# Streampunk/phaneron

Hardware: AMD Instinct MI355X
Metric: frames/sec, 4-layer 2160p50 composite pipeline (v210 unpack->CSC->combine->CSC->v210 pack) (higher is better)
Workload: dtype f32

## Files before the change

include/phaneron_hip.h:

```cpp
#ifndef PHANERON_HIP_H
#define PHANERON_HIP_H

#include <stddef.h>
#include <stdint.h>

#ifdef __cplusplus
extern "C" {
#endif

#define PH_ABI_VERSION 8

enum {
  PH_OK = 0,
  PH_E_INVALID = -1,
  PH_E_NO_DEVICE = -2,
  PH_E_HIP = -3,
  PH_E_UNKNOWN_KERNEL = -4,
  PH_E_RANGE = -5
};

typedef struct ph_ctx ph_ctx;
typedef struct ph_buf ph_buf;
typedef struct ph_program ph_program;

// ... 248 lines not shown
int ph_chan_compose_multi(ph_ctx *ctx, int queue, int n, const ph_chan_layer *layers, int n_out, const ph_chan_output *outs,
                          uint32_t out_width, uint32_t out_height, const void *rd_col_matrix12, const void *rd_gamma_lut,
                          const void *rd_gamut9);
int ph_compose_up_write_multi(ph_ctx *ctx, int queue, int jobs, int n, const ph_image_layer *const *layer_sets, int n_out,
                              const ph_chan_output *outs, uint32_t out_width, uint32_t out_height);

int ph_lut_register(ph_ctx *ctx, const void *device_lut_f32, const float *host_lut65536);
int ph_lut_unregister(ph_ctx *ctx, const void *device_lut_f32);
int ph_lut_query(ph_ctx *ctx, const void *device_lut_f32, uint32_t *lds_bytes, uint32_t *index_bias,
                 uint32_t *blocks_per_octave_log2);
typedef struct ph_lut_layout {
  uint32_t lds_bytes, hole, delta_off, shift, index_bias;
  float a_scale;
} ph_lut_layout;
int ph_lut_layout_of(const float *host_lut65536, ph_lut_layout *layout, void *lds_image, size_t capacity);
int ph_ctx_set_option(ph_ctx *ctx, const char *name, int value);

int ph_colour_gamma2linear_lut(const char *colspec, float *lut65536);
int ph_colour_linear2gamma_lut(const char *colspec, float *lut65536);
int ph_colour_ycbcr2rgb_matrix(const char *colspec, int num_bits, int luma_black, int luma_white,
                               int chroma_range, float *m12);
int ph_colour_rgb2ycbcr_matrix(const char *colspec, int num_bits, int luma_black, int luma_white,
                               int chroma_range, float *m12);
int ph_colour_rgb2rgb_matrix(const char *src_colspec, const char *dst_colspec, float *m9);
int ph_transform_matrix(int width, int height, int flip_h, int flip_v, double anchor_x,
                        double anchor_y, double scale_x, double scale_y, double offset_x,
                        double offset_y, double rotate, float *m9);

int ph_abi_version(void);

// ... 5 lines not shown
```

phaneron_amd/capi.py:

```python
import ctypes as C
import os
import sys

import numpy as np

_HERE = os.path.dirname(os.path.abspath(__file__))
LIB_PATH = os.environ.get("PHANERON_HIP_LIB") or os.path.join(_HERE, "lib", "libphaneron_hip.so")

QUEUE_LOAD, QUEUE_PROCESS, QUEUE_UNLOAD = 0, 1, 2
HOST_READONLY, HOST_WRITEONLY, HOST_NONE = 0, 1, 2
ARG_BUF, ARG_U32, ARG_I32, ARG_F32 = 0, 1, 2, 3

EXPORTS = [
    "ph_abi_version", "ph_last_error", "ph_ctx_create", "ph_ctx_destroy", "ph_ctx_info", "ph_ctx_stream",
    "ph_wait_finish", "ph_buf_create", "ph_buf_wrap", "ph_buf_addref", "ph_buf_release", "ph_buf_refcount",
    "ph_buf_bytes", "ph_buf_device_ptr", "ph_buf_dims", "ph_buf_host_access", "ph_buf_host_ptr",
    "ph_ctx_buffer_stats", "ph_program_create", "ph_program_destroy", "ph_program_kernel", "ph_run_program", "ph_check_program", "ph_chan_compose", "ph_yadif_pair_packed",
    "ph_v210_pitch_bytes", "ph_v210_read", "ph_v210_read_batch", "ph_v210_write", "ph_yadif", "ph_yadif_pair", "ph_v210_yadif_pair", "ph_transform", "ph_resize", "ph_combine",
    "ph_transition_dissolve", "ph_transition_wipe", "ph_mixer", "ph_wipe", "ph_fused_v210_combine",
    "ph_colour_gamma2linear_lut", "ph_colour_linear2gamma_lut", "ph_colour_ycbcr2rgb_matrix",
    "ph_colour_rgb2ycbcr_matrix", "ph_colour_rgb2rgb_matrix", "ph_transform_matrix",
    "ph_lut_register", "ph_lut_unregister", "ph_lut_query", "ph_lut_layout_of", "ph_compose_up_write_v210_pair", "ph_compose_up_write_v210_batch", "ph_pack_read_batch", "ph_ctx_set_option", "ph_compose_write_v210", "ph_compose_wipe_write_v210",
    "ph_pack_plane_bytes", "ph_pack_read", "ph_pack_write", "ph_queue_wait_queue", "ph_buf_download_async",
    "ph_event_record", "ph_event_wait", "ph_event_query", "ph_event_destroy", "ph_queue_query",
    "ph_graph_begin", "ph_graph_end", "ph_graph_launch", "ph_graph_destroy", "ph_fused_v210_combine_batch",
    "ph_program_resolve", "ph_route_unique_id", "ph_route_init", "ph_route_destroy", "ph_route_group_begin",
    "ph_route_group_end", "ph_route_send", "ph_route_recv", "ph_route_after_queue", "ph_queue_after_route",
    "ph_route_wait", "ph_route_stream", "ph_route_comm_count", "ph_chan_compose_v210", "ph_chan_compose_batch", "ph_run_programs", "ph_event_record_timed", "ph_event_elapsed_us", "ph_ctx_host_pool_stats",
    "ph_v210_yadif_pair_fmt", "ph_compose_up_write_v210", "ph_trace_begin", "ph_trace_end", "ph_run_programs_progress", "ph_buf_reuse", "ph_image_unpack_rgb",
    "ph_chan_compose_multi", "ph_compose_up_write_multi",
]


class PhaneronError(RuntimeError):
    pass


class _ArgVal(C.Union):
    _fields_ = [("buf", C.c_void_p), ("u32", C.c_uint32), ("i32", C.c_int32), ("f32", C.c_float)]


class PhArg(C.Structure):
    _fields_ = [("name", C.c_char_p), ("kind", C.c_int), ("v", _ArgVal)]


# ... 117 lines not shown
        "ph_transition_wipe": (ci, [vp, ci, vp, vp, vp, ci, ci, vp]),
        "ph_mixer": (ci, [vp, ci, vp, vp, cf, ci, ci, vp]),
        "ph_wipe": (ci, [vp, ci, vp, vp, cf, ci, ci, vp]),
        "ph_fused_v210_combine": (ci, [vp, ci, ci, C.POINTER(vp), vp, cu, cu, vp, vp, vp, vp, vp]),
        "ph_fused_v210_combine_batch": (ci, [vp, ci, ci, ci, C.POINTER(vp), C.POINTER(vp), cu, cu, vp, vp, vp, vp, vp]),
        "ph_colour_gamma2linear_lut": (ci, [C.c_char_p, f32p]),
        "ph_colour_linear2gamma_lut": (ci, [C.c_char_p, f32p]),
        "ph_colour_ycbcr2rgb_matrix": (ci, [C.c_char_p, ci, ci, ci, ci, f32p]),
        "ph_colour_rgb2ycbcr_matrix": (ci, [C.c_char_p, ci, ci, ci, ci, f32p]),
        "ph_colour_rgb2rgb_matrix": (ci, [C.c_char_p, C.c_char_p, f32p]),
        "ph_transform_matrix": (ci, [ci, ci, ci, ci, cd, cd, cd, cd, cd, cd, cd, f32p]),
        "ph_lut_register": (ci, [vp, vp, f32p]),
        "ph_lut_unregister": (ci, [vp, vp]),
        "ph_lut_query": (ci, [vp, vp, C.POINTER(cu), C.POINTER(cu), C.POINTER(cu)]),
        "ph_lut_layout_of": (ci, [f32p, C.POINTER(LutLayout), vp, C.c_size_t]),
        "ph_compose_up_write_v210_pair": (ci, [vp, ci, ci, C.POINTER(PhImageLayer), C.POINTER(PhImageLayer), vp, vp, cu, cu, cu, vp, vp]),
        "ph_compose_up_write_v210_batch": (ci, [vp, ci, ci, ci, C.POINTER(C.POINTER(PhImageLayer)), C.POINTER(vp), cu, cu, cu, vp, vp]),
        "ph_pack_read_batch": (ci, [vp, ci, ci, ci, C.POINTER(vp * 3), C.POINTER(vp), cu, cu, vp, vp, vp]),
        "ph_ctx_set_option": (ci, [vp, C.c_char_p, ci]),
        "ph_pack_plane_bytes": (ci, [ci, cu, cu, C.POINTER(cs)]),
        "ph_pack_read": (ci, [vp, ci, ci, C.POINTER(vp), vp, cu, cu, vp, vp, vp]),
        "ph_pack_write": (ci, [vp, ci, ci, vp, C.POINTER(vp), cu, cu, cu, vp, vp]),
        "ph_compose_write_v210": (ci, [vp, ci, ci, C.POINTER(PhLayer), vp, cu, cu, cu, vp, vp]),
        "ph_compose_wipe_write_v210": (ci, [vp, ci, ci, C.POINTER(PhLayer), C.POINTER(PhLayerWipe), vp, cu, cu, cu, vp, vp]),
        "ph_compose_up_write_v210": (ci, [vp, ci, ci, C.POINTER(PhImageLayer), vp, cu, cu, cu, vp, vp]),
        "ph_chan_compose_v210": (ci, [vp, ci, ci, C.POINTER(PhChanLayer), vp, cu, cu, cu, vp, vp, vp, vp, vp]),
        "ph_chan_compose": (ci, [vp, ci, ci, C.POINTER(PhChanLayer), ci, C.POINTER(C.c_void_p), cu, cu, cu, vp, vp, vp, vp, vp]),
        "ph_chan_compose_batch": (ci, [vp, ci, ci, C.POINTER(PhChanJob), cu, cu, vp, vp, vp, vp, vp]),
        "ph_chan_compose_multi": (ci, [vp, ci, ci, C.POINTER(PhChanLayer), ci, C.POINTER(PhChanOutput), cu, cu, vp, vp, vp]),
        "ph_compose_up_write_multi": (ci, [vp, ci, ci, ci, C.POINTER(C.POINTER(PhImageLayer)), ci, C.POINTER(PhChanOutput), cu, cu]),
# ... 57 lines not shown
def lut_layout(lut):
    lut = np.ascontiguousarray(lut, np.float32)
    assert lut.shape == (65536,)
    lay = LutLayout()
    n = lib().ph_lut_layout_of(lut, C.byref(lay), None, 0)
    if n < 0:
        check(n)
    if n == 0:
        return None, None
    image = np.zeros(n, np.uint8)
    if lib().ph_lut_layout_of(lut, C.byref(lay), image.ctypes.data_as(C.c_void_p), n) != n:
        check(-1)
    return {k: getattr(lay, k) for k, _ in LutLayout._fields_}, image


def gamma2linear_lut(colspec):
    out = np.empty(65536, np.float32)
    check(lib().ph_colour_gamma2linear_lut(colspec.encode(), out))
    return out


def linear2gamma_lut(colspec):
    out = np.empty(65536, np.float32)
    check(lib().ph_colour_linear2gamma_lut(colspec.encode(), out))
    return out


def ycbcr2rgb_matrix(colspec, num_bits=10, luma_black=64, luma_white=940, chroma_range=896):
    out = np.empty(12, np.float32)
    check(lib().ph_colour_ycbcr2rgb_matrix(colspec.encode(), num_bits, luma_black, luma_white, chroma_range, out))
# ... 659 lines not shown
```

phaneron_amd/csrc/ph_api.cpp:

```cpp
#include <atomic>
#include <chrono>
#include <cstdarg>
#include <cstdio>
#include <cstring>
#include <dlfcn.h>
#include <map>
#include <mutex>
#include <string>
#include <vector>

#include "../../include/phaneron_hip.h"
#include "ph_internal.h"
#include "ph_kernels.h"
#include "ph_lut_host.h"

using ph::KernelId;
using namespace ph;

namespace {
thread_local std::string g_err;
}

int fail(int code, const char *fmt, ...) {
  char buf[512];
// ... 831 lines not shown
int ph_lut_layout_of(const float *host, ph_lut_layout *layout, void *lds_image, size_t capacity) {
  if (!host || !layout) return fail(PH_E_INVALID, "ph_lut_layout_of: NULL argument");
  std::vector<uint32_t> blob;
  ph::LutHostInfo info;
  memset(layout, 0, sizeof(*layout));
  if (!ph::lut_compress(host, ph::kLutMaxLdsBytes, blob, info)) return 0;
  const ph::LutView v = ph::lut_view(info, nullptr);
  layout->lds_bytes = info.bytes, layout->hole = info.hole, layout->delta_off = info.delta_off, layout->shift = info.shift;
  layout->index_bias = (uint32_t)info.bias, layout->a_scale = v.a_scale;
  if (lds_image) {
    if (capacity < info.bytes) return fail(PH_E_INVALID, "ph_lut_layout_of: the image needs %u bytes, %zu given", info.bytes, capacity);
    memset(lds_image, 0, info.hole);
    memcpy(static_cast<char *>(lds_image) + info.hole, blob.data(), info.bytes - info.hole);
  }
  return (int)info.bytes;
}

int ph_lut_query(ph_ctx *ctx, const void *dev, uint32_t *lds_bytes, uint32_t *toe, uint32_t *shift) {
  if (!ctx) return fail(PH_E_INVALID, "ph_lut_query: ctx is NULL");
  std::lock_guard<std::mutex> lock(ctx->mu);
  auto it = ctx->luts.find(dev);
  const bool have = it != ctx->luts.end();
  if (lds_bytes) *lds_bytes = have ? it->second.view.bytes : 0;
  if (toe) *toe = have ? (uint32_t)it->second.view.bias : 0;
  if (shift) *shift = have ? 23 - it->second.view.shift : 0;
  return PH_OK;
}

int ph_ctx_set_option(ph_ctx *ctx, const char *name, int value) {
  if (!ctx || !name) return fail(PH_E_INVALID, "ph_ctx_set_option: NULL argument");
// ... 1205 lines not shown
```

phaneron_amd/csrc/ph_kernels.h:

```cpp
#pragma once
#include <hip/hip_runtime.h>
#include <stddef.h>
#include <stdint.h>

#include "ph_formats.h"
#include "ph_lut.h"

namespace ph {

constexpr int kMaxLayers = 8;
constexpr int kMaxDynamicLds = 160 * 1024;

extern thread_local uint32_t t_stream_images;
extern thread_local uint32_t t_stream_threshold_mb;
static inline uint32_t image_nt(size_t bytes) {
  return t_stream_images == 2 ? (bytes > ((size_t)t_stream_threshold_mb << 20) ? 1u : 0u) : t_stream_images;
}

struct FusedArgs {
  const void *layers[kMaxLayers];
  void *out;
  uint32_t quads_per_line_used;
  uint32_t quads_per_line_pitch;
  uint32_t total_quads;
  const float *rd_cm, *rd_lut, *rd_gm, *wr_cm, *wr_lut;
  uint32_t tail_px, magic_qpp;
};

constexpr int kMaxBatch = 8;
struct FusedLdsArgs {
  FusedArgs f;
  LutView rd, wr;
  uint32_t jobs, wg_per_job;
  const void *more_layers[kMaxBatch - 1][kMaxLayers];
  void *more_out[kMaxBatch - 1];
};

struct ComposeArgs {
  const void *layers[kMaxLayers];
  const float *matrix[kMaxLayers];
  const void *wipe_with[kMaxLayers], *wipe_mask[kMaxLayers];
  int lw[kMaxLayers], lh[kMaxLayers];
  int n;
  void *out;
  uint32_t out_w, out_h, lines, first_line, line_step;
  const float *wr_cm;
  LutView wr;
};

enum : uint32_t { kChanNone = 0, kChanV210 = 1, kChanRgba = 2, kChanP10 = 3, kChanP8x422 = 4, kChanP8x420 = 5, kChanNv12 = 6, kChanP10x420 = 7,
                  kChanP010 = 8, kChanRgba8 = 9, kChanBgra8 = 10, kChanPlanarLast = kChanP010 };
// ... 215 lines not shown
```

phaneron_amd/csrc/ph_kernels_deint.hip:

```cpp
#include "ph_device.h"
#include "ph_kernels.h"
#include "ph_ldslut.h"
#include "ph_yadif.h"

#include <type_traits>

#pragma clang fp contract(off)

namespace ph {

constexpr int kDeintCols = 64 - 6;
#ifndef PH_DEINT_BLOCK
#define PH_DEINT_BLOCK 1024
#endif
constexpr int kDeintBlock = PH_DEINT_BLOCK;

struct Rgb {
  float r, g, b;
};

struct LanePick {
  uint32_t off_y, off_cb, off_cr;
  uint32_t sy, scb, scr;
};
// ... 51 lines not shown

__device__ __forceinline__ float lane_tap(float v, uint32_t lane, int d) {
  return __int_as_float(__builtin_amdgcn_ds_bpermute((int)((lane + (uint32_t)d) << 2), __float_as_int(v)));
}

#define PH_RGB(v, c) ((c) == 0 ? (v).r : (c) == 1 ? (v).g : (v).b)
#ifndef PH_DEINT_PRICE_INDEX
#define PH_DEINT_PRICE_INDEX 0
#endif

template <int TFF, bool STD, int PACK = PH_FMT_V210>
__device__ __forceinline__ void v210_yadif_pair_body(const DeintArgs &a, const ReadK &k, const LutK &lk) {
  const uint32_t wave = __builtin_amdgcn_readfirstlane(threadIdx.x >> 6), lane = threadIdx.x & 63;
  const int w = (int)a.width, h = (int)a.height;
  const uint32_t tasks = (uint32_t)a.n * a.strips * a.col_blocks;
  for (uint32_t t = blockIdx.x * (kDeintBlock / 64) + wave; t < tasks; t += gridDim.x * (kDeintBlock / 64)) {
    const uint32_t cb = t % a.col_blocks, rest = t / a.col_blocks, strip = rest % a.strips, l = rest / a.strips;
    constexpr bool V210 = PACK == PH_FMT_V210;
    const uint32_t line_bytes = V210 ? a.quads_pitch * 16u : a.quads_pitch * (fmt_wide(PACK) ? 2u : 1u);
    const int frame_bytes = (int)(line_bytes * a.height);
    auto planes = [&](const uint4 *y, const void *u, const void *v) __attribute__((always_inline)) {
      FramePlanes f;
      f.y = __builtin_amdgcn_make_buffer_rsrc(const_cast<uint4 *>(y), 0, frame_bytes, 0x00020000);
      if (fmt_cbcr(PACK)) {
        f.u = f.v = __builtin_amdgcn_make_buffer_rsrc(const_cast<void *>(u), 0, (int)(line_bytes * ((a.height + 1u) >> 1)), 0x00020000);
      } else if (!V210) {
        const int chroma_bytes = fmt_v420(PACK) ? (int)((line_bytes >> 1) * ((a.height + 1u) >> 1)) : frame_bytes / 2;
        f.u = __builtin_amdgcn_make_buffer_rsrc(const_cast<void *>(u), 0, chroma_bytes, 0x00020000);
        f.v = __builtin_amdgcn_make_buffer_rsrc(const_cast<void *>(v), 0, chroma_bytes, 0x00020000);
      } else {
        f.u = f.v = f.y;
// ... 92 lines not shown
hipError_t launch_v210_yadif_pair(hipStream_t s, DeintArgs a, int tff, uint32_t num_cus) {
  const uint32_t slots = num_cus * (kDeintBlock / 64);
  a.col_blocks = (a.width + kDeintCols - 1) / kDeintCols;
  uint32_t best_r = 16;
  uint64_t best_cost = ~0ull;
  for (uint32_t r = 8; r <= 64; r += 2) {
    const uint32_t strips = (a.height + r - 1) / r;
    const uint64_t tasks = (uint64_t)a.n * strips * a.col_blocks, rounds = (tasks + slots - 1) / slots;
    const uint64_t cost = rounds * (r + 4);
    if (cost < best_cost) best_cost = cost, best_r = r;
  }
  a.nt = image_nt((size_t)a.width * a.height * (a.rgb12 ? 12 : 16));
  a.rows_per_strip = best_r;
  a.strips = (a.height + best_r - 1) / best_r;
  const uint32_t tasks = (uint32_t)a.n * a.strips * a.col_blocks;
  const uint32_t want = (tasks + kDeintBlock / 64 - 1) / (kDeintBlock / 64);
  const uint32_t grid = want < num_cus ? want : num_cus;
  auto go = [&](auto kernel) -> hipError_t {
    hipError_t e = hipFuncSetAttribute(reinterpret_cast<const void *>(kernel), hipFuncAttributeMaxDynamicSharedMemorySize, kMaxDynamicLds);
    if (e != hipSuccess) return e;
    kernel<<<grid, kDeintBlock, a.lut.bytes, s>>>(a);
    return hipGetLastError();
  };
  switch (a.pack) {
    case PH_FMT_V210: return tff ? go(v210_yadif_pair_kernel<1, PH_FMT_V210>) : go(v210_yadif_pair_kernel<0, PH_FMT_V210>);
    case PH_FMT_YUV422P10: return tff ? go(v210_yadif_pair_kernel<1, PH_FMT_YUV422P10>) : go(v210_yadif_pair_kernel<0, PH_FMT_YUV422P10>);
    case PH_FMT_YUV422P8: return tff ? go(v210_yadif_pair_kernel<1, PH_FMT_YUV422P8>) : go(v210_yadif_pair_kernel<0, PH_FMT_YUV422P8>);
    case PH_FMT_YUV420P: return tff ? go(v210_yadif_pair_kernel<1, PH_FMT_YUV420P>) : go(v210_yadif_pair_kernel<0, PH_FMT_YUV420P>);
    case PH_FMT_NV12: return tff ? go(v210_yadif_pair_kernel<1, PH_FMT_NV12>) : go(v210_yadif_pair_kernel<0, PH_FMT_NV12>);
  }
  return hipErrorInvalidValue;
}
// ... 3 lines not shown
```

phaneron_amd/csrc/ph_kernels_fmt.hip:

```cpp
#include <cstdlib>
#include <type_traits>

#include "ph_kernels.h"
#include "ph_ldslut.h"

#pragma clang fp contract(off)

namespace ph {

constexpr int kFmtBlock = 256;

template <typename LUT>
__device__ __forceinline__ float4 yuv_to_rgba(float y, float u, float v, const ReadK &k, const LUT &lut) {
  const float r = lut.at_unit(dot4(y, u, v, 1.0f, k.r));
  const float g = lut.at_unit(dot4(y, u, v, 1.0f, k.g));
  const float b = lut.at_unit(dot4(y, u, v, 1.0f, k.b));
  return make_float4(dot3(r, g, b, k.gm[0], k.gm[1], k.gm[2]), dot3(r, g, b, k.gm[3], k.gm[4], k.gm[5]),
                     dot3(r, g, b, k.gm[6], k.gm[7], k.gm[8]), 1.0f);
}

struct FmtReadArgs {
  const void *p0, *p1, *p2;
  float4 *out;
  uint32_t width, lines, pitch;
// ... 86 lines not shown
      const float4 px = a.in[(size_t)line * a.width + x];
      const float r = lut.at_unit(px.x), gg = lut.at_unit(px.y), b = lut.at_unit(px.z);
      const uint32_t r8 = sat_u8_rte(r * 255.0f);
      const uint32_t g8 = sat_u8_rte(gg * 255.0f);
      const uint32_t b8 = sat_u8_rte(b * 255.0f);
      const uint32_t w = FMT == PH_FMT_RGBA8 ? (r8 | g8 << 8 | b8 << 16 | 0xff000000u) : (b8 | g8 << 8 | r8 << 16 | 0xff000000u);
      reinterpret_cast<uint32_t *>(a.p0)[(size_t)line * a.pitch + x] = w;
    }
    return;
  }
  constexpr bool V420 = fmt_v420(FMT), WIDE = fmt_wide(FMT);
  constexpr uint32_t MSB = fmt_msb(FMT);
  const WriteK k = load_write_k(a.cm);
  const uint32_t full = a.width / 8, remain = a.width % 8, octets = full + (remain ? 1 : 0);
  const uint32_t total = octets * a.groups;
  const uint32_t stride = PERSISTENT ? gridDim.x * blockDim.x : total;
  for (uint32_t f = blockIdx.x * blockDim.x + threadIdx.x; f < total; f += stride) {
    const uint32_t g = f / octets, o8 = f - g * octets;
    const bool tail = (o8 == full);
    const uint32_t n = tail ? (remain < 6 ? remain : 6) : 8;
    const uint32_t first = V420 ? g * 2 + ((3 == a.interlace) ? 1 : 0)
                                : g * (a.interlace ? 2 : 1) + ((3 == a.interlace) ? 1 : 0);
    const uint32_t nlines = V420 ? (a.interlace ? 1 : 2) : 1;
    const uint32_t crow = V420 ? g : first;
    for (uint32_t l = 0; l < nlines; ++l) {
      const uint32_t line = first + l;
      const float4 *px = a.in + (size_t)line * a.width + 8 * o8;
      uint32_t y[8], u[4], v[4];
#pragma unroll
      for (int p = 0; p < 8; ++p) y[p] = WIDE ? 64u : 16u;
#pragma unroll
      for (int p = 0; p < 4; ++p) u[p] = v[p] = WIDE ? 512u : 128u;
// ... 132 lines not shown
  b.cm = (const float *)cm, b.gm = (const float *)gm, b.nt = image_nt((size_t)width * height * 16);
  return for_fmt(fmt, [&](auto f) { return launch_read_batch_fmt<decltype(f)::value>(s, b, lv, num_cus); });
}

template <int FMT>
static hipError_t launch_write_fmt(hipStream_t s, const FmtWriteArgs &a, const float *table, const LutView *lv,
                                   uint32_t num_cus) {
  const bool rgb = fmt_rgb8(FMT);
  const uint32_t total = rgb ? a.width * a.groups : ((a.width + 7) / 8) * a.groups;
  if (!total) return hipSuccess;
  if (lv) {
    hipError_t e = hipFuncSetAttribute(reinterpret_cast<const void *>(fmt_write_lds_kernel<FMT>),
                                       hipFuncAttributeMaxDynamicSharedMemorySize, kMaxDynamicLds);
    if (e != hipSuccess) return e;
    const uint32_t want = (total + kLdsBlock - 1) / kLdsBlock;
    fmt_write_lds_kernel<FMT><<<want < num_cus ? want : num_cus, kLdsBlock, lv->bytes, s>>>(a, *lv);
  } else {
    fmt_write_gather_kernel<FMT><<<(total + kFmtBlock - 1) / kFmtBlock, kFmtBlock, 0, s>>>(a, table);
  }
  return hipGetLastError();
}

hipError_t launch_pack_write(hipStream_t s, int fmt, const void *in, void *const planes[3], uint32_t width,
                             uint32_t height, uint32_t interlace, const void *cm, const void *table, const LutView *lv,
                             uint32_t num_cus) {
  const bool v420 = fmt_v420(fmt);
  const uint32_t groups = v420 ? height / 2 : (interlace ? height / 2 : height);
  FmtWriteArgs a{(const float4 *)in, planes[0], planes[1], planes[2], width, pack_pitch(fmt, width), groups, interlace,
                 (const float *)cm};
  return for_fmt(fmt, [&](auto f) { return launch_write_fmt<decltype(f)::value>(s, a, (const float *)table, lv, num_cus); });
}
// ... 3 lines not shown
```

phaneron_amd/csrc/ph_kernels_lds.hip:

```cpp
#include "ph_device.h"
#include "ph_kernels.h"
#include "ph_ldslut.h"

#include <cstdlib>

#include <type_traits>

#pragma clang fp contract(off)

#ifndef PH_PROBE
#define PH_PROBE 0
#endif
#if PH_PROBE
__device__ unsigned long long g_fused_probe[2048 * 12];
extern "C" int ph_debug_fused_probe(unsigned long long *out, int n_words) {
  return (int)hipMemcpyFromSymbol(out, HIP_SYMBOL(g_fused_probe), (size_t)n_words * 8);
}
#define PH_STAMP(k)                                                                  \
  do {                                                                               \
    if (threadIdx.x == 0 && tile_begin == wg_begin) {                                \
      g_fused_probe[blockIdx.x * 12 + 2 * (k)] = __builtin_amdgcn_s_memtime();       \
      g_fused_probe[blockIdx.x * 12 + 2 * (k) + 1] = __builtin_amdgcn_s_memrealtime(); \
    }                                                                                \
  } while (0)
// ... 36 lines not shown
}

#ifndef PH_FUSED_SPLIT
#define PH_FUSED_SPLIT 0
#endif
template <int N, int P, int BS, bool PIPE = false, int MODE = 0, bool TAIL = false>
__global__ __launch_bounds__(BS) void fused_v210_combine_lds_kernel(FusedLdsArgs a, uint32_t *handoff = nullptr) {
  static_assert(!TAIL || (!PIPE && MODE == 0), "the tail instantiation exists for the shipped form only");
  const ReadK rk = load_read_k(a.f.rd_cm, a.f.rd_gm);
  const WriteK wk = load_write_k(a.f.wr_cm);
  const LutK rlut = make_lut_k(a.rd), wlut = make_lut_k(a.wr);
  const bool std_matrix = ycbcr_matrix_is_standard(rk);
  const uint32_t job = blockIdx.x / a.wg_per_job, wg_in_job = blockIdx.x - job * a.wg_per_job;
  auto layer_ptr = [&](int l) { return reinterpret_cast<const uint4 *>(job ? a.more_layers[job - 1][l] : a.f.layers[l]); };
  uint4 *const out_ptr = reinterpret_cast<uint4 *>(job ? a.more_out[job - 1] : a.f.out);
  const uint32_t per_wg = (a.f.total_quads + a.wg_per_job - 1) / a.wg_per_job;
  const uint32_t wg_begin = wg_in_job * per_wg;
  const uint32_t wg_end = wg_begin + per_wg < a.f.total_quads ? wg_begin + per_wg : a.f.total_quads;
  const uint32_t tile_quads = BS * P;
  for (uint32_t tile_begin = wg_begin; tile_begin < wg_end; tile_begin += tile_quads) {
    uint32_t st[P][9];
    auto quad_of = [&](int p) {
      const uint32_t f = tile_begin + p * BS + threadIdx.x;
      return f < wg_end ? f : wg_end - 1;
    };
    uint4 w = load_stream(layer_ptr(0) + quad_of(0));
    auto slot_kind = [&](uint32_t f) -> uint32_t {
      const uint32_t g = f - __umulhi(f, a.f.magic_qpp) * a.f.quads_per_line_pitch;
      return g < a.f.quads_per_line_used ? 0u : (g == a.f.quads_per_line_used && a.f.tail_px) ? 1u : 2u;
    };
    auto phase1_slice = [&](auto tag, uint4 w, uint32_t f, uint32_t f_next, bool more, uint32_t(&st)[9]) -> uint4 {
      const bool in_tail = TAIL && slot_kind(f) == 1u;
      const float last = TAIL ? (in_tail ? 0.0f : 1.0f) : 1.0f;
// ... 255 lines not shown
    const float crf = (float)((wcr >> scr) & 0x3ff);
    store_image(out + p, read_px_lds(yf, cbf, crf, k, lk, x < tail_from ? 1.0f : 0.0f), nt);
  }
}

__global__ __launch_bounds__(kLdsBlock) void v210_write_lds_kernel(const float4 *__restrict__ in, uint4 *__restrict__ out,
                                                                    uint32_t width, uint32_t quads_per_line,
                                                                    uint32_t lines, uint32_t first_line,
                                                                    uint32_t line_step, const float *__restrict__ cm,
                                                                    LutView lut) {
  const WriteK k = load_write_k(cm);
  const LutK lk = make_lut_k(lut);
  lds_lut_load(lut);
  __syncthreads();
  const uint32_t total = quads_per_line * lines, full = width / 6u, remain = width - 6u * full;
  for (uint32_t f = blockIdx.x * kLdsBlock + threadIdx.x; f < total; f += gridDim.x * kLdsBlock) {
    const uint32_t li = f / quads_per_line, g = f - li * quads_per_line;
    const uint32_t line = first_line + li * line_step;
    if (g > full || (g == full && !remain)) {
      store_stream(out + (size_t)line * quads_per_line + g, make_uint4(0u, 0u, 0u, 0u));
      continue;
    }
    const float4 *row = in + (size_t)line * width;
    float rgb[18];
#pragma unroll
    for (int j = 0; j < 6; ++j) {
      const uint32_t x = 6u * g + (uint32_t)j < width ? 6u * g + (uint32_t)j : width - 1u;
      const float4 p = row[x];
      rgb[3 * j] = p.x, rgb[3 * j + 1] = p.y, rgb[3 * j + 2] = p.z;
    }
    if (g == full) {
// ... 2 lines not shown
      for (int i = 0; i < 18; ++i) yi[i] = lds_lut_index_unit_tail(rgb[i], true);
      store_stream(out + (size_t)line * quads_per_line + g, write_quad_idx_lds_tail(yi, k, lk, remain));
      continue;
    }
    store_stream(out + (size_t)line * quads_per_line + g, write_quad_lds(rgb, k, lk));
  }
}

__global__ __launch_bounds__(kLdsBlock) void compose_write_v210_kernel(ComposeArgs a) {
  const WriteK wk = load_write_k(a.wr_cm);
  const LutK lk = make_lut_k(a.wr);
  lds_lut_load(a.wr);
  __syncthreads();
  const uint32_t qpl = (a.out_w + 47u) / 48u * 8u, full = a.out_w / 6u, remain = a.out_w - 6u * full;
  const uint32_t total = qpl * a.lines;
  for (uint32_t f = blockIdx.x * kLdsBlock + threadIdx.x; f < total; f += gridDim.x * kLdsBlock) {
    const uint32_t li = f / qpl, g = f - li * qpl;
    const uint32_t line = a.first_line + li * a.line_step;
    if (g > full || (g == full && !remain)) {
      store_stream(reinterpret_cast<uint4 *>(a.out) + (size_t)line * qpl + g, make_uint4(0u, 0u, 0u, 0u));
      continue;
    }
    float acc[24];
#pragma unroll 1
    for (int l = 0; l < a.n; ++l) {
      const float4 *img = reinterpret_cast<const float4 *>(a.layers[l]);
      const int lw = a.lw[l], lh = a.lh[l];
      const float *m = a.matrix[l];
      float m0 = 0, m1 = 0, m2 = 0, m3 = 0, m4 = 0, m5 = 0;
      if (m) m0 = m[0], m1 = m[1], m2 = m[2], m3 = m[3], m4 = m[4], m5 = m[5];
      const float py = (float)(int)line / (float)(int)a.out_h - 0.5f;
// ... 43 lines not shown
  float mm[N][6];
  bool direct[N];
#pragma unroll
  for (int l = 0; l < N; ++l) {
    direct[l] = a.matrix[l] == nullptr;
#pragma unroll
    for (int i = 0; i < 6; ++i) mm[l][i] = direct[l] ? 0.0f : a.matrix[l][i];
  }
  lds_lut_load(a.wr);
  __syncthreads();
  const uint32_t wave = threadIdx.x >> 6, lane = threadIdx.x & 63;
  uint16_t *ys = reinterpret_cast<uint16_t *>(g_lds + stage_off + wave * kComposeChunk * 4);
  uint16_t *us = ys + kComposeChunk, *vs = us + kComposeChunk / 2;
  const uint32_t qpl = a.out_w / 6;
  const uint32_t total_px = a.out_w * a.lines;
  const uint32_t waves_total = gridDim.x * (kLdsBlock / 64);
  for (uint32_t base = (blockIdx.x * (kLdsBlock / 64) + wave) * kComposeChunk; base < total_px;
       base += waves_total * kComposeChunk) {
#pragma unroll 1
    for (uint32_t k = 0; k < kComposeChunk / 64; ++k) {
      const uint32_t local = k * 64 + lane;
      uint32_t p = base + local;
      p = p < total_px ? p : total_px - 1;
      const uint32_t li = p / a.out_w, x = p - li * a.out_w;
      const uint32_t line = a.first_line + li * a.line_step;
      const float py = (float)(int)line / (float)(int)a.out_h - 0.5f;
      const float px = (float)(int)x / (float)(int)a.out_w - 0.5f;
      float4 t[N];
#pragma unroll
      for (int l = 0; l < N; ++l) {
        if (ALL_DIRECT) {
          t[l] = load_stream(reinterpret_cast<const float4 *>(a.layers[l]) + (size_t)line * a.out_w + x);
// ... 311 lines not shown
}
#endif

template <int N, int P, int BS, bool PIPE = false, bool TAIL = false>
static hipError_t launch_fused_npb(hipStream_t s, const FusedLdsArgs &a, uint32_t grid_in, uint32_t lds) {
  uint32_t grid = grid_in;
#if PH_FUSED_SPLIT
  static const int cus_env = [] {
    const char *e = getenv("PH_FUSED_CUS");
    return e ? atoi(e) : 0;
  }();
  if (cus_env > 0 && (uint32_t)cus_env < grid) grid = (uint32_t)cus_env;
#endif
  hipError_t e = allow_lds(fused_v210_combine_lds_kernel<N, P, BS, PIPE, 0, TAIL>, lds);
  if (e != hipSuccess) return e;
  const uint32_t slices = (a.f.total_quads + BS - 1) / BS;
  FusedLdsArgs b = a;
  if (b.jobs < 1) b.jobs = 1;
  b.wg_per_job = grid / b.jobs ? grid / b.jobs : 1;
  if (b.wg_per_job > slices) b.wg_per_job = slices;
#if PH_FUSED_SPLIT
  if (!PIPE && N == 4) {
    static const int mode_env = [] {
      const char *e = getenv("PH_FUSED_MODE");
      return e ? atoi(e) : 0;
    }();
    if (mode_env == 1) return launch_fused_half<N, P, BS, 1>(s, b, lds);
    if (mode_env == 2) return launch_fused_half<N, P, BS, 2>(s, b, lds);
    if (mode_env == 3) {
      hipError_t e1 = launch_fused_half<N, P, BS, 1>(s, b, lds);
      return e1 != hipSuccess ? e1 : launch_fused_half<N, P, BS, 2>(s, b, lds);
    }
  }
#endif
  fused_v210_combine_lds_kernel<N, P, BS, PIPE, 0, TAIL><<<b.wg_per_job * b.jobs, BS, lds, s>>>(b);
// ... 38 lines not shown
    case 7: return launch_fused_n<7>(s, a, num_cus, lds);
    case 8: return launch_fused_n<8>(s, a, num_cus, lds);
    default: return hipErrorInvalidValue;
  }
}

hipError_t launch_compose_write_v210(hipStream_t s, const ComposeArgs &a, uint32_t num_cus) {
  const uint32_t total = (a.out_w + 47u) / 48u * 8u * a.lines;
  if (!total) return hipSuccess;
  bool any_wipe = false;
  for (int l = 0; l < a.n; ++l) any_wipe = any_wipe || a.wipe_with[l] != nullptr;
  if (any_wipe && !compose_uses_taps(a)) return hipErrorInvalidValue;
  const uint32_t stage_off = (a.wr.bytes + 15u) & ~15u;
  if (!compose_quad_forced() && compose_stage_fits(a) && a.out_w % 48u == 0) {
    const uint32_t chunks = (a.out_w * a.lines + kComposeChunk - 1) / kComposeChunk;
    const uint32_t want = (chunks + kLdsBlock / 64 - 1) / (kLdsBlock / 64);
    const uint32_t grid = want < num_cus ? want : num_cus;
    if (compose_uses_taps(a)) {
      switch (a.n) {
        case 1: return launch_compose_taps_n<1>(s, a, grid, stage_off);
        case 2: return launch_compose_taps_n<2>(s, a, grid, stage_off);
        case 3: return launch_compose_taps_n<3>(s, a, grid, stage_off);
        case 4: return launch_compose_taps_n<4>(s, a, grid, stage_off);
        case 5: return launch_compose_taps_n<5>(s, a, grid, stage_off);
        case 6: return launch_compose_taps_n<6>(s, a, grid, stage_off);
        case 7: return launch_compose_taps_n<7>(s, a, grid, stage_off);
        case 8: return launch_compose_taps_n<8>(s, a, grid, stage_off);
        default: return hipErrorInvalidValue;
      }
    }
    switch (a.n) {
      case 1: return launch_compose_px_n<1>(s, a, grid, stage_off);
      case 2: return launch_compose_px_n<2>(s, a, grid, stage_off);
      case 3: return launch_compose_px_n<3>(s, a, grid, stage_off);
      case 4: return launch_compose_px_n<4>(s, a, grid, stage_off);
      case 5: return launch_compose_px_n<5>(s, a, grid, stage_off);
      case 6: return launch_compose_px_n<6>(s, a, grid, stage_off);
      case 7: return launch_compose_px_n<7>(s, a, grid, stage_off);
      case 8: return launch_compose_px_n<8>(s, a, grid, stage_off);
      default: return hipErrorInvalidValue;
    }
  }
  hipError_t e = allow_lds(compose_write_v210_kernel, a.wr.bytes);
  if (e != hipSuccess) return e;
  const uint32_t want = (total + kLdsBlock - 1) / kLdsBlock;
  compose_write_v210_kernel<<<want < num_cus ? want : num_cus, kLdsBlock, a.wr.bytes, s>>>(a);
  return hipGetLastError();
}

__global__ void lds_base_probe_kernel(uint32_t *out) {
  *out = (uint32_t)(uintptr_t)(__attribute__((address_space(3))) unsigned char *)g_lds;
}
hipError_t launch_lds_base_probe(hipStream_t s, uint32_t *out_dev) {
  lds_base_probe_kernel<<<1, 64, 16, s>>>(out_dev);
  return hipGetLastError();
}

hipError_t launch_v210_read_lds(hipStream_t s, const void *in, void *out, uint32_t width, uint32_t height,
                                const void *cm, const void *gm, const LutView &lut, uint32_t num_cus) {
  hipError_t e = allow_lds(v210_read_lds_kernel, lut.bytes);
  if (e != hipSuccess) return e;
// ... 16 lines not shown
  uint32_t per = num_cus / (uint32_t)n ? num_cus / (uint32_t)n : 1;
  a.wg_per_frame = want < per ? want : per;
  v210_read_lds_batch_kernel<<<a.wg_per_frame * n, kLdsBlock, lut.bytes, s>>>(a, width, v210_pitch_bytes(width) / 16, total,
                                                                              (const float *)cm, (const float *)gm, lut,
                                                                              image_nt((size_t)width * height * 16));
  return hipGetLastError();
}

hipError_t launch_v210_write_lds(hipStream_t s, const void *in, void *out, uint32_t width, uint32_t height,
                                 uint32_t interlace, const void *cm, const LutView &lut, uint32_t num_cus) {
  hipError_t e = allow_lds(v210_write_lds_kernel, lut.bytes);
  if (e != hipSuccess) return e;
  const uint32_t step = interlace ? 2 : 1, first = (interlace == 3) ? 1 : 0;
  const uint32_t lines = interlace ? height / 2 : height, qpl = v210_pitch_bytes(width) / 16;
  if (!lines) return hipSuccess;
  const uint32_t want = (qpl * lines + kLdsBlock - 1) / kLdsBlock;
  v210_write_lds_kernel<<<want < num_cus ? want : num_cus, kLdsBlock, lut.bytes, s>>>(
      (const float4 *)in, (uint4 *)out, width, qpl, lines, first, step, (const float *)cm, lut);
  return hipGetLastError();
}

}
```

phaneron_amd/csrc/ph_kernels_up.hip:

```cpp
#include "ph_device.h"
#include "ph_kernels.h"
#include "ph_ldslut.h"

#include <cstdlib>
#include <type_traits>

#pragma clang fp contract(off)

#ifndef PH_UP_GROUP_ROWS
#define PH_UP_GROUP_ROWS 16
#endif

namespace ph {

#ifndef PH_UP_BLOCK
#define PH_UP_BLOCK 1024
#endif
constexpr int kUpBlock = PH_UP_BLOCK;
constexpr uint32_t kUpCols = 126;
constexpr uint32_t kUpOutside = 0x40000000u;

typedef uint32_t ph_u32x3 __attribute__((ext_vector_type(3)));
typedef uint32_t ph_u32x4 __attribute__((ext_vector_type(4)));

// ... 741 lines not shown
  return rgb12 ? go(clip_up_write_v210_kernel<true, false, false>) : go(clip_up_write_v210_kernel<false, false, false>);
}

bool compose_up_eligible(const UpArgs &a) {
  if (a.out_w % 2u || !a.n) return false;
  for (int l = 0; l < a.n; ++l) {
    const UpLayer &L = a.layer[l];
    if (L.m[1] != 0.0f || L.m[3] != 0.0f || !(L.m[0] > 0.0f) || !(L.m[4] > 0.0f)) return false;
    const bool fill = L.w == a.out_w && L.h == a.out_h && a.line_step == 1u && L.m[0] == 1.0f && L.m[4] == 1.0f && L.m[2] == 0.0f && L.m[5] == 0.0f;
    if (!fill && ((double)L.m[0] * L.w > 0.99 * a.out_w || (double)L.m[4] * L.h * a.line_step > 0.99 * a.out_h)) return false;
    if ((uint64_t)L.pitch * L.h >= (1ull << 30) || L.w >= (1u << 22)) return false;
  }
  return true;
}

static uint32_t up_plan(UpArgs &b, bool tails, uint32_t num_cus, uint32_t cols = kUpCols) {
  if (!b.jobs) b.jobs = 1;
  b.out_qpitch = v210_pitch_bytes(b.out_w) / 16u;
  b.cover_w = tails ? b.out_qpitch * 6u : b.out_w;
  b.shared = 1;
  for (int l = 1; l < b.n; ++l) {
    b.shared = b.shared && b.layer[l].w == b.layer[0].w && b.layer[l].h == b.layer[0].h && b.layer[l].pitch == b.layer[0].pitch;
    for (int k = 0; k < 6; ++k) b.shared = b.shared && b.layer[l].m[k] == b.layer[0].m[k];
  }
  const uint32_t upr = (b.cover_w + cols - 1u) / cols, upg = (uint32_t)(PH_UP_GROUP_ROWS / 2) * upr;
  const uint32_t units = upr * ((b.lines + 1u) / 2u) * b.jobs;
  b.magic_upr = upr > 1 ? (uint32_t)(((1ull << 32) + upr - 1) / upr) : 0u;
  b.magic_upg = (uint32_t)(((1ull << 32) + upg - 1) / upg);
  const uint32_t want = (units + kUpBlock / 64 - 1) / (kUpBlock / 64);
  return want < num_cus ? want : num_cus;
}

hipError_t launch_compose_up_write_v210(hipStream_t s, const UpArgs &a, bool rgb12, uint32_t num_cus) {
  if (!a.lines) return hipSuccess;
  const bool tails = a.out_w % 48u != 0;
  const void *fn = tails ? (rgb12 ? reinterpret_cast<const void *>(compose_up_write_v210_kernel<true, true>)
                                  : reinterpret_cast<const void *>(compose_up_write_v210_kernel<false, true>))
                         : (rgb12 ? reinterpret_cast<const void *>(compose_up_write_v210_kernel<true>)
                                  : reinterpret_cast<const void *>(compose_up_write_v210_kernel<false>));
  hipError_t e = hipFuncSetAttribute(fn, hipFuncAttributeMaxDynamicSharedMemorySize, kMaxDynamicLds);
  if (e != hipSuccess) return e;
  UpArgs b = a;
  const uint32_t grid = up_plan(b, tails, num_cus);
  if (tails && rgb12) compose_up_write_v210_kernel<true, true><<<grid, kUpBlock, a.wr.bytes, s>>>(b);
  else if (tails) compose_up_write_v210_kernel<false, true><<<grid, kUpBlock, a.wr.bytes, s>>>(b);
  else if (rgb12) compose_up_write_v210_kernel<true><<<grid, kUpBlock, a.wr.bytes, s>>>(b);
  else compose_up_write_v210_kernel<false><<<grid, kUpBlock, a.wr.bytes, s>>>(b);
  return hipGetLastError();
}

hipError_t launch_compose_up_multi(hipStream_t s, const UpMultiArgs &m, bool rgb12, uint32_t num_cus) {
  if (!m.up.lines) return hipSuccess;
  if (m.n_out < 1 || m.n_out > (uint32_t)kMaxUpOuts || m.up.jobs < 1 || m.up.jobs > (uint32_t)kMaxUpJobs) return hipErrorInvalidValue;
  for (uint32_t k = 0; k < m.n_out; ++k)
    if (!fmt_chan_out((int)m.out[k].fmt) || (m.out[k].fmt == PH_FMT_V210 && m.up.out_w % 48u)) return hipErrorInvalidValue;
  char name[48];
  snprintf(name, sizeof name, "compose_up_multi<%s>x%uj%u", rgb12 ? "rgb" : "rgba", m.n_out, m.up.jobs);
  if (trace_launch(name)) return hipSuccess;
// ... 18 lines not shown
```

Before: 19970.

## Spread small table-kernel work across more CUs and balance fused per-workgroup quad shares

Grid sizing for several LDS-table kernels changes: instead of packing work into as few full blocks as possible, the grid is sized to one wave of work per CU (up to the CU count), and each block enables only as many lanes or waves as its share needs, with the rest exiting early. The fused v210 combine kernel gets a helper that computes workgroups per job so quad shares are even and no workgroup is left empty. The aim is to use more CUs on small launches, at the cost of loading the LDS table in more blocks. A debug API that exposes the share computation is also added.

```diff
diff --git a/include/phaneron_hip.h b/include/phaneron_hip.h
--- a/include/phaneron_hip.h
+++ b/include/phaneron_hip.h
@@ -286,6 +286,7 @@
   float a_scale;
 } ph_lut_layout;
 int ph_lut_layout_of(const float *host_lut65536, ph_lut_layout *layout, void *lds_image, size_t capacity);
+int ph_debug_fused_shares(uint32_t total_quads, uint32_t num_cus, uint32_t jobs, uint32_t wg_per_job, uint32_t *begins, uint32_t *ends);
 int ph_ctx_set_option(ph_ctx *ctx, const char *name, int value);
 
 int ph_colour_gamma2linear_lut(const char *colspec, float *lut65536);
diff --git a/phaneron_amd/capi.py b/phaneron_amd/capi.py
--- a/phaneron_amd/capi.py
+++ b/phaneron_amd/capi.py
@@ -28,7 +28,7 @@
     "ph_route_group_end", "ph_route_send", "ph_route_recv", "ph_route_after_queue", "ph_queue_after_route",
     "ph_route_wait", "ph_route_stream", "ph_route_comm_count", "ph_chan_compose_v210", "ph_chan_compose_batch", "ph_run_programs", "ph_event_record_timed", "ph_event_elapsed_us", "ph_ctx_host_pool_stats",
     "ph_v210_yadif_pair_fmt", "ph_compose_up_write_v210", "ph_trace_begin", "ph_trace_end", "ph_run_programs_progress", "ph_buf_reuse", "ph_image_unpack_rgb",
-    "ph_chan_compose_multi", "ph_compose_up_write_multi",
+    "ph_chan_compose_multi", "ph_compose_up_write_multi", "ph_debug_fused_shares",
 ]
 
 
@@ -176,6 +176,7 @@
         "ph_lut_unregister": (ci, [vp, vp]),
         "ph_lut_query": (ci, [vp, vp, C.POINTER(cu), C.POINTER(cu), C.POINTER(cu)]),
         "ph_lut_layout_of": (ci, [f32p, C.POINTER(LutLayout), vp, C.c_size_t]),
+        "ph_debug_fused_shares": (ci, [cu, cu, cu, cu, C.POINTER(cu), C.POINTER(cu)]),
         "ph_compose_up_write_v210_pair": (ci, [vp, ci, ci, C.POINTER(PhImageLayer), C.POINTER(PhImageLayer), vp, vp, cu, cu, cu, vp, vp]),
         "ph_compose_up_write_v210_batch": (ci, [vp, ci, ci, ci, C.POINTER(C.POINTER(PhImageLayer)), C.POINTER(vp), cu, cu, cu, vp, vp]),
         "ph_pack_read_batch": (ci, [vp, ci, ci, ci, C.POINTER(vp * 3), C.POINTER(vp), cu, cu, vp, vp, vp]),
@@ -263,6 +264,17 @@
     return {k: getattr(lay, k) for k, _ in LutLayout._fields_}, image
 
 
+def fused_shares(total_quads, wg_per_job=0, num_cus=256, jobs=1):
+    n = lib().ph_debug_fused_shares(total_quads, num_cus, jobs, wg_per_job, None, None)
+    if n < 0:
+        check(n)
+    begins, ends = np.empty(n, np.uint32), np.empty(n, np.uint32)
+    u32p = C.POINTER(C.c_uint32)
+    if lib().ph_debug_fused_shares(total_quads, num_cus, jobs, n, begins.ctypes.data_as(u32p), ends.ctypes.data_as(u32p)) != n:
+        check(-1)
+    return begins, ends
+
+
 def gamma2linear_lut(colspec):
     out = np.empty(65536, np.float32)
     check(lib().ph_colour_gamma2linear_lut(colspec.encode(), out))
diff --git a/phaneron_amd/csrc/ph_api.cpp b/phaneron_amd/csrc/ph_api.cpp
--- a/phaneron_amd/csrc/ph_api.cpp
+++ b/phaneron_amd/csrc/ph_api.cpp
@@ -869,6 +869,17 @@
     memcpy(static_cast<char *>(lds_image) + info.hole, blob.data(), info.bytes - info.hole);
   }
   return (int)info.bytes;
+}
+
+int ph_debug_fused_shares(uint32_t total_quads, uint32_t num_cus, uint32_t jobs, uint32_t wg_per_job, uint32_t *begins, uint32_t *ends) {
+  if (!total_quads || jobs < 1 || jobs > (uint32_t)ph::kMaxBatch) return fail(PH_E_INVALID, "ph_debug_fused_shares: no quads, or not 1..%d jobs", ph::kMaxBatch);
+  if (!wg_per_job) wg_per_job = ph::fused_wg_per_job(total_quads, num_cus, jobs);
+  if ((uint64_t)total_quads + wg_per_job > 0xFFFFFFFFull) return fail(PH_E_INVALID, "ph_debug_fused_shares: %u quads are more than a launch takes", total_quads);
+  for (uint32_t wg = 0; begins && ends && wg < wg_per_job; ++wg) {
+    const ph::QuadShare s = ph::fused_share(total_quads, wg_per_job, wg);
+    begins[wg] = s.begin, ends[wg] = s.end;
+  }
+  return (int)wg_per_job;
 }
 
 int ph_lut_query(ph_ctx *ctx, const void *dev, uint32_t *lds_bytes, uint32_t *toe, uint32_t *shift) {
diff --git a/phaneron_amd/csrc/ph_kernels.h b/phaneron_amd/csrc/ph_kernels.h
--- a/phaneron_amd/csrc/ph_kernels.h
+++ b/phaneron_amd/csrc/ph_kernels.h
@@ -35,6 +35,30 @@
   const void *more_layers[kMaxBatch - 1][kMaxLayers];
   void *more_out[kMaxBatch - 1];
 };
+
+__host__ __device__ inline uint32_t fused_wg_per_job(uint32_t total_quads, uint32_t grid, uint32_t jobs) {
+  const uint32_t share = grid / (jobs ? jobs : 1u), waves = (total_quads + 63u) / 64u;
+  const uint32_t most = share < waves ? share : waves, wg = most ? most : 1u;
+  const uint32_t per = (total_quads + wg - 1u) / wg;
+  return per ? (total_quads + per - 1u) / per : 1u;
+}
+struct QuadShare {
+  uint32_t begin, end;
+};
+__host__ __device__ inline QuadShare fused_share(uint32_t total_quads, uint32_t wg_per_job, uint32_t wg) {
+  const uint32_t per_wg = (total_quads + wg_per_job - 1u) / wg_per_job;
+  const uint32_t from = wg * per_wg, begin = from < total_quads ? from : total_quads;
+  return {begin, per_wg < total_quads - begin ? begin + per_wg : total_quads};
+}
+
+static inline uint32_t table_kernel_grid(uint32_t units, uint32_t num_cus) {
+  const uint32_t waves = (units + 63u) / 64u, grid = waves < num_cus ? waves : num_cus;
+  return grid ? grid : 1u;
+}
+__host__ __device__ inline uint32_t table_kernel_lanes(uint32_t units, uint32_t grid, uint32_t block) {
+  const uint32_t per = (units + grid - 1u) / grid, lanes = (per + 63u) & ~63u;
+  return lanes < block ? lanes : block;
+}
 
 struct ComposeArgs {
   const void *layers[kMaxLayers];
diff --git a/phaneron_amd/csrc/ph_kernels_deint.hip b/phaneron_amd/csrc/ph_kernels_deint.hip
--- a/phaneron_amd/csrc/ph_kernels_deint.hip
+++ b/phaneron_amd/csrc/ph_kernels_deint.hip
@@ -89,7 +89,9 @@
   const uint32_t wave = __builtin_amdgcn_readfirstlane(threadIdx.x >> 6), lane = threadIdx.x & 63;
   const int w = (int)a.width, h = (int)a.height;
   const uint32_t tasks = (uint32_t)a.n * a.strips * a.col_blocks;
-  for (uint32_t t = blockIdx.x * (kDeintBlock / 64) + wave; t < tasks; t += gridDim.x * (kDeintBlock / 64)) {
+  const uint32_t wpw = table_kernel_lanes(tasks * 64u, gridDim.x, kDeintBlock) / 64u;
+  if (wave >= wpw) return;
+  for (uint32_t t = blockIdx.x * wpw + wave; t < tasks; t += gridDim.x * wpw) {
     const uint32_t cb = t % a.col_blocks, rest = t / a.col_blocks, strip = rest % a.strips, l = rest / a.strips;
     constexpr bool V210 = PACK == PH_FMT_V210;
     const uint32_t line_bytes = V210 ? a.quads_pitch * 16u : a.quads_pitch * (fmt_wide(PACK) ? 2u : 1u);
@@ -212,8 +214,7 @@
   a.rows_per_strip = best_r;
   a.strips = (a.height + best_r - 1) / best_r;
   const uint32_t tasks = (uint32_t)a.n * a.strips * a.col_blocks;
-  const uint32_t want = (tasks + kDeintBlock / 64 - 1) / (kDeintBlock / 64);
-  const uint32_t grid = want < num_cus ? want : num_cus;
+  const uint32_t grid = tasks < num_cus ? tasks : num_cus;
   auto go = [&](auto kernel) -> hipError_t {
     hipError_t e = hipFuncSetAttribute(reinterpret_cast<const void *>(kernel), hipFuncAttributeMaxDynamicSharedMemorySize, kMaxDynamicLds);
     if (e != hipSuccess) return e;
diff --git a/phaneron_amd/csrc/ph_kernels_fmt.hip b/phaneron_amd/csrc/ph_kernels_fmt.hip
--- a/phaneron_amd/csrc/ph_kernels_fmt.hip
+++ b/phaneron_amd/csrc/ph_kernels_fmt.hip
@@ -124,8 +124,10 @@
   const WriteK k = load_write_k(a.cm);
   const uint32_t full = a.width / 8, remain = a.width % 8, octets = full + (remain ? 1 : 0);
   const uint32_t total = octets * a.groups;
-  const uint32_t stride = PERSISTENT ? gridDim.x * blockDim.x : total;
-  for (uint32_t f = blockIdx.x * blockDim.x + threadIdx.x; f < total; f += stride) {
+  const uint32_t lanes = PERSISTENT ? table_kernel_lanes(total, gridDim.x, blockDim.x) : blockDim.x;
+  const uint32_t stride = PERSISTENT ? gridDim.x * lanes : total;
+  if (PERSISTENT && threadIdx.x >= lanes) return;
+  for (uint32_t f = blockIdx.x * lanes + threadIdx.x; f < total; f += stride) {
     const uint32_t g = f / octets, o8 = f - g * octets;
     const bool tail = (o8 == full);
     const uint32_t n = tail ? (remain < 6 ? remain : 6) : 8;
@@ -288,7 +290,7 @@
                                        hipFuncAttributeMaxDynamicSharedMemorySize, kMaxDynamicLds);
     if (e != hipSuccess) return e;
     const uint32_t want = (total + kLdsBlock - 1) / kLdsBlock;
-    fmt_write_lds_kernel<FMT><<<want < num_cus ? want : num_cus, kLdsBlock, lv->bytes, s>>>(a, *lv);
+    fmt_write_lds_kernel<FMT><<<rgb ? (want < num_cus ? want : num_cus) : table_kernel_grid(total, num_cus), kLdsBlock, lv->bytes, s>>>(a, *lv);
   } else {
     fmt_write_gather_kernel<FMT><<<(total + kFmtBlock - 1) / kFmtBlock, kFmtBlock, 0, s>>>(a, table);
   }
diff --git a/phaneron_amd/csrc/ph_kernels_lds.hip b/phaneron_amd/csrc/ph_kernels_lds.hip
--- a/phaneron_amd/csrc/ph_kernels_lds.hip
+++ b/phaneron_amd/csrc/ph_kernels_lds.hip
@@ -74,9 +74,8 @@
   const uint32_t job = blockIdx.x / a.wg_per_job, wg_in_job = blockIdx.x - job * a.wg_per_job;
   auto layer_ptr = [&](int l) { return reinterpret_cast<const uint4 *>(job ? a.more_layers[job - 1][l] : a.f.layers[l]); };
   uint4 *const out_ptr = reinterpret_cast<uint4 *>(job ? a.more_out[job - 1] : a.f.out);
-  const uint32_t per_wg = (a.f.total_quads + a.wg_per_job - 1) / a.wg_per_job;
-  const uint32_t wg_begin = wg_in_job * per_wg;
-  const uint32_t wg_end = wg_begin + per_wg < a.f.total_quads ? wg_begin + per_wg : a.f.total_quads;
+  const QuadShare share = fused_share(a.f.total_quads, a.wg_per_job, wg_in_job);
+  const uint32_t wg_begin = share.begin, wg_end = share.end;
   const uint32_t tile_quads = BS * P;
   for (uint32_t tile_begin = wg_begin; tile_begin < wg_end; tile_begin += tile_quads) {
     uint32_t st[P][9];
@@ -362,7 +361,9 @@
   lds_lut_load(lut);
   __syncthreads();
   const uint32_t total = quads_per_line * lines, full = width / 6u, remain = width - 6u * full;
-  for (uint32_t f = blockIdx.x * kLdsBlock + threadIdx.x; f < total; f += gridDim.x * kLdsBlock) {
+  const uint32_t lanes = table_kernel_lanes(total, gridDim.x, kLdsBlock);
+  if (threadIdx.x >= lanes) return;
+  for (uint32_t f = blockIdx.x * lanes + threadIdx.x; f < total; f += gridDim.x * lanes) {
     const uint32_t li = f / quads_per_line, g = f - li * quads_per_line;
     const uint32_t line = first_line + li * line_step;
     if (g > full || (g == full && !remain)) {
@@ -395,7 +396,9 @@
   __syncthreads();
   const uint32_t qpl = (a.out_w + 47u) / 48u * 8u, full = a.out_w / 6u, remain = a.out_w - 6u * full;
   const uint32_t total = qpl * a.lines;
-  for (uint32_t f = blockIdx.x * kLdsBlock + threadIdx.x; f < total; f += gridDim.x * kLdsBlock) {
+  const uint32_t lanes = table_kernel_lanes(total, gridDim.x, kLdsBlock);
+  if (threadIdx.x >= lanes) return;
+  for (uint32_t f = blockIdx.x * lanes + threadIdx.x; f < total; f += gridDim.x * lanes) {
     const uint32_t li = f / qpl, g = f - li * qpl;
     const uint32_t line = a.first_line + li * a.line_step;
     if (g > full || (g == full && !remain)) {
@@ -469,8 +472,10 @@
   uint16_t *us = ys + kComposeChunk, *vs = us + kComposeChunk / 2;
   const uint32_t qpl = a.out_w / 6;
   const uint32_t total_px = a.out_w * a.lines;
-  const uint32_t waves_total = gridDim.x * (kLdsBlock / 64);
-  for (uint32_t base = (blockIdx.x * (kLdsBlock / 64) + wave) * kComposeChunk; base < total_px;
+  const uint32_t wpw = table_kernel_lanes((total_px + kComposeChunk - 1) / kComposeChunk * 64u, gridDim.x, kLdsBlock) / 64u;
+  if (wave >= wpw) return;
+  const uint32_t waves_total = gridDim.x * wpw;
+  for (uint32_t base = (blockIdx.x * wpw + wave) * kComposeChunk; base < total_px;
        base += waves_total * kComposeChunk) {
 #pragma unroll 1
     for (uint32_t k = 0; k < kComposeChunk / 64; ++k) {
@@ -812,11 +817,9 @@
 #endif
   hipError_t e = allow_lds(fused_v210_combine_lds_kernel<N, P, BS, PIPE, 0, TAIL>, lds);
   if (e != hipSuccess) return e;
-  const uint32_t slices = (a.f.total_quads + BS - 1) / BS;
   FusedLdsArgs b = a;
   if (b.jobs < 1) b.jobs = 1;
-  b.wg_per_job = grid / b.jobs ? grid / b.jobs : 1;
-  if (b.wg_per_job > slices) b.wg_per_job = slices;
+  b.wg_per_job = fused_wg_per_job(a.f.total_quads, grid, b.jobs);
 #if PH_FUSED_SPLIT
   if (!PIPE && N == 4) {
     static const int mode_env = [] {
@@ -885,9 +888,8 @@
   const uint32_t stage_off = (a.wr.bytes + 15u) & ~15u;
   if (!compose_quad_forced() && compose_stage_fits(a) && a.out_w % 48u == 0) {
     const uint32_t chunks = (a.out_w * a.lines + kComposeChunk - 1) / kComposeChunk;
-    const uint32_t want = (chunks + kLdsBlock / 64 - 1) / (kLdsBlock / 64);
-    const uint32_t grid = want < num_cus ? want : num_cus;
     if (compose_uses_taps(a)) {
+      const uint32_t want = (chunks + kLdsBlock / 64 - 1) / (kLdsBlock / 64), grid = want < num_cus ? want : num_cus;
       switch (a.n) {
         case 1: return launch_compose_taps_n<1>(s, a, grid, stage_off);
         case 2: return launch_compose_taps_n<2>(s, a, grid, stage_off);
@@ -900,6 +902,7 @@
         default: return hipErrorInvalidValue;
       }
     }
+    const uint32_t grid = chunks < num_cus ? chunks : num_cus;
     switch (a.n) {
       case 1: return launch_compose_px_n<1>(s, a, grid, stage_off);
       case 2: return launch_compose_px_n<2>(s, a, grid, stage_off);
@@ -914,8 +917,7 @@
   }
   hipError_t e = allow_lds(compose_write_v210_kernel, a.wr.bytes);
   if (e != hipSuccess) return e;
-  const uint32_t want = (total + kLdsBlock - 1) / kLdsBlock;
-  compose_write_v210_kernel<<<want < num_cus ? want : num_cus, kLdsBlock, a.wr.bytes, s>>>(a);
+  compose_write_v210_kernel<<<table_kernel_grid(total, num_cus), kLdsBlock, a.wr.bytes, s>>>(a);
   return hipGetLastError();
 }
 
@@ -962,8 +964,7 @@
   const uint32_t step = interlace ? 2 : 1, first = (interlace == 3) ? 1 : 0;
   const uint32_t lines = interlace ? height / 2 : height, qpl = v210_pitch_bytes(width) / 16;
   if (!lines) return hipSuccess;
-  const uint32_t want = (qpl * lines + kLdsBlock - 1) / kLdsBlock;
-  v210_write_lds_kernel<<<want < num_cus ? want : num_cus, kLdsBlock, lut.bytes, s>>>(
+  v210_write_lds_kernel<<<table_kernel_grid(qpl * lines, num_cus), kLdsBlock, lut.bytes, s>>>(
       (const float4 *)in, (uint4 *)out, width, qpl, lines, first, step, (const float *)cm, lut);
   return hipGetLastError();
 }
diff --git a/phaneron_amd/csrc/ph_kernels_up.hip b/phaneron_amd/csrc/ph_kernels_up.hip
--- a/phaneron_amd/csrc/ph_kernels_up.hip
+++ b/phaneron_amd/csrc/ph_kernels_up.hip
@@ -779,7 +779,7 @@
   return true;
 }
 
-static uint32_t up_plan(UpArgs &b, bool tails, uint32_t num_cus, uint32_t cols = kUpCols) {
+static uint32_t up_plan(UpArgs &b, bool tails, uint32_t num_cus, uint32_t cols = kUpCols, bool spread = false) {
   if (!b.jobs) b.jobs = 1;
   b.out_qpitch = v210_pitch_bytes(b.out_w) / 16u;
   b.cover_w = tails ? b.out_qpitch * 6u : b.out_w;
@@ -792,7 +792,7 @@
   const uint32_t units = upr * ((b.lines + 1u) / 2u) * b.jobs;
   b.magic_upr = upr > 1 ? (uint32_t)(((1ull << 32) + upr - 1) / upr) : 0u;
   b.magic_upg = (uint32_t)(((1ull << 32) + upg - 1) / upg);
-  const uint32_t want = (units + kUpBlock / 64 - 1) / (kUpBlock / 64);
+  const uint32_t want = spread ? units : (units + kUpBlock / 64 - 1) / (kUpBlock / 64);
   return want < num_cus ? want : num_cus;
 }
 
@@ -806,7 +806,7 @@
   hipError_t e = hipFuncSetAttribute(fn, hipFuncAttributeMaxDynamicSharedMemorySize, kMaxDynamicLds);
   if (e != hipSuccess) return e;
   UpArgs b = a;
-  const uint32_t grid = up_plan(b, tails, num_cus);
+  const uint32_t grid = up_plan(b, tails, num_cus, kUpCols, !tails);
   if (tails && rgb12) compose_up_write_v210_kernel<true, true><<<grid, kUpBlock, a.wr.bytes, s>>>(b);
   else if (tails) compose_up_write_v210_kernel<false, true><<<grid, kUpBlock, a.wr.bytes, s>>>(b);
   else if (rgb12) compose_up_write_v210_kernel<true><<<grid, kUpBlock, a.wr.bytes, s>>>(b);
```

Result: no change. 19940 (median of 3 runs) (-0.1%).
